# chto/linna

Measured on AMD Instinct MI355X. Metric: emulator log-likelihood evals/sec, higher is better.
Workload: dtype f32; 1 GPU; 33-D Gaussian, 4x512 MLP emulator (33->512x4->33), nwalkers=4096 batched log-likelihood per GPU (BASELINE configs[1]); nwalkers_per_gpu=4096, launch=direct launches, parallelism=walkers sharded, 1 rank(s), no data-path collective

## Files before the change

### include/linna_hip.h

```cpp
#ifndef LINNA_HIP_H
#define LINNA_HIP_H
#include <stddef.h>
#include <stdint.h>

#ifdef __cplusplus
extern "C" {
#endif

#define LINNA_ABI_VERSION 12

typedef struct linna_ctx linna_ctx_t;
typedef struct linna_net linna_net_t;
typedef struct linna_logprob linna_logprob_t;
typedef struct linna_graph linna_graph_t;

int linna_abi_version(void);
const char* linna_last_error(void);
#define LINNA_OK 0
#define LINNA_ERR_INVALID (-1)
#define LINNA_ERR_HIP (-2)
#define LINNA_ERR_UNSUPPORTED (-3)
#define LINNA_ERR_INTERNAL (-4)
int linna_debug_raise(int kind);
int linna_ctx_create(int device, linna_ctx_t** out);
// ... 119 lines not shown
    linna_colmap_t outmap;
    const float* S; int lds;
    const float* Ssym;
    const float* w;
    const float* gscale;
    float temperature;
    const float* Sfac;
} linna_logprob_desc_t;

int linna_logprob_create(linna_ctx_t* ctx, linna_net_t* net, const linna_logprob_desc_t* desc,
                         linna_logprob_t** out);
int linna_logprob_destroy(linna_logprob_t* lp);
int linna_weights_changed(linna_ctx_t* ctx);
#define LINNA_PRECISION_FP32 0
#define LINNA_PRECISION_BF16 1
int linna_logprob_set_precision(linna_logprob_t* lp, int precision);
int linna_logprob_precision(const linna_logprob_t* lp, int* out);
int linna_logprob_set_grad_precision(linna_logprob_t* lp, int precision);
int linna_logprob_grad_precision(const linna_logprob_t* lp, int* out);
int linna_engine_rows(int rows);
int linna_dense_tri(int mode);
int linna_serve_plain(int on);
int linna_serve_plain_sched(int hand);
int linna_program_plain(const linna_layer_t* layers, int nlayers, int in_size, int rows, int dense_nout);
int linna_logprob_serve_plain(linna_logprob_t* lp, int B, int* out);
int linna_logprob_grad_launches(linna_logprob_t* lp, int B, int* out);
int linna_slice_fusion(int mask);
int linna_program_describe(const linna_layer_t* layers, int nlayers, int in_size, int rows, int dense_nout, char* buf,
                           size_t n);
int linna_program_describe_grad_bf16(const linna_layer_t* layers, int nlayers, int in_size, int rows, char* buf, size_t n);
size_t linna_logprob_ws_bytes(const linna_logprob_t* lp, int B, int with_grad);
int linna_logprob_eval(linna_logprob_t* lp, const float* Z, int ldz, int B, void* ws, float* lnP,
                       float* THETA, int ldt, void* stream);
int linna_logprob_eval_if(linna_logprob_t* lp, const float* Z, int ldz, int B, void* ws, float* lnP,
                          float* THETA, int ldt, const int* gate, void* stream);
int linna_logprob_eval_slice_points(linna_logprob_t* lp, const float* coords, int ldc, int ndim, const int* S_idx,
                                    int ns, const float* DIR, int ldd, const float* w, int nrep, float* lnP,
                                    const int* gate, void* stream);
int linna_logprob_grad(linna_logprob_t* lp, const float* Z, int ldz, int B, void* ws, float* lnP,
                       float* G, int ldg, void* stream);
int linna_logprob_grad_leapfrog(linna_logprob_t* lp, float* Q, int ldq, int B, void* ws, float* lnP, float* G, int ldg,
                                float* P, int ldp, const float* mass, float eps_kick, float eps_drift, void* stream);

typedef struct {
    uint32_t struct_size;
    int nout;
// ... 165 lines not shown
```

### linna_amd/_lib.py

```python
import ctypes as C
import os

import torch

_HERE = os.path.dirname(os.path.abspath(__file__))
LIB_PATH = os.environ.get("LINNA_LIB_PATH") or os.path.join(_HERE, "liblinna_hip.so")
ABI_VERSION = 12

c_float_p = C.c_void_p
c_int_p = C.c_void_p


class _Sized(C.Structure):

    def __init__(self, *a, **k):
        C.Structure.__init__(self, *a, **k)
        self.struct_size = C.sizeof(type(self))


def sized_array(cls, n):
    arr = (cls * n)()
    for i in range(n):
        arr[i].struct_size = C.sizeof(cls)
    return arr
# ... 83 lines not shown
    "linna_net_create": (_I, [_V, C.POINTER(Layer), _I, _I, _PV]),
    "linna_net_destroy": (_I, [_V]),
    "linna_net_prepare": (_I, [_V, _I, _I]),
    "linna_net_fwd_ws_bytes": (_SZ, [_V, _I]),
    "linna_net_bwd_ws_bytes": (_SZ, [_V, _I]),
    "linna_net_forward": (_I, [_V, _V, _I, _I, _V, _V, _I, C.POINTER(ColMap), _V]),
    "linna_net_backward": (_I, [_V, _V, _I, _I, _V, _V, _V, _I, _V, _I, _I, _V]),
    "linna_net_stream_state": (_I, [_V, _V, _V, _V]),
    "linna_prior_map_fwd": (_I, [_V, _V, _I, _I, _I, _V, _V, _V, _V, _V, _V, _V, _I, _V, _I, _V]),
    "linna_prior_map_bwd": (_I, [_V, _V, _I, _I, _I, _V, _V, _V, _V, _V, _V, _I, _V, _I, _V]),
    "linna_gauss_loglike_diag": (_I, [_V, _V, _I, _I, _I, _V, _V, _I, _I, _F, _V, _V]),
    "linna_gauss_loglike_dense": (_I, [_V, _V, _I, _I, _I, _V, _I, _V, _I, _I, _F, _V, _V, _V]),
    "linna_logprob_create": (_I, [_V, _V, C.POINTER(LogprobDesc), _PV]),
    "linna_logprob_destroy": (_I, [_V]),
    "linna_weights_changed": (_I, [_V]),
    "linna_logprob_set_precision": (_I, [_V, _I]),
    "linna_logprob_precision": (_I, [_V, _V]),
    "linna_logprob_set_grad_precision": (_I, [_V, _I]),
    "linna_logprob_grad_precision": (_I, [_V, _V]),
    "linna_engine_rows": (_I, [_I]),
    "linna_dense_tri": (_I, [_I]),
    "linna_serve_plain": (_I, [_I]),
    "linna_serve_plain_sched": (_I, [_I]),
    "linna_program_plain": (_I, [_V, _I, _I, _I, _I]),
    "linna_logprob_serve_plain": (_I, [_V, _I, _V]),
    "linna_logprob_grad_launches": (_I, [_V, _I, _V]),
    "linna_slice_fusion": (_I, [_I]),
    "linna_net_train_launches": (_I, [_V, _I]),
    "linna_net_set_train_precision": (_I, [_V, _I]),
    "linna_net_train_precision": (_I, [_V, _V]),
    "linna_program_describe": (_I, [_V, _I, _I, _I, _I, _V, C.c_size_t]),
    "linna_program_describe_grad_bf16": (_I, [_V, _I, _I, _I, _V, C.c_size_t]),
    "linna_logprob_ws_bytes": (_SZ, [_V, _I, _I]),
    "linna_logprob_eval": (_I, [_V, _V, _I, _I, _V, _V, _V, _I, _V]),
    "linna_logprob_grad": (_I, [_V, _V, _I, _I, _V, _V, _V, _I, _V]),
    "linna_logprob_grad_leapfrog": (_I, [_V, _V, _I, _I, _V, _V, _V, _I, _V, _I, _V, _F, _F, _V]),
    "linna_loss_scratch_bytes": (_SZ, [_I, _I]),
    "linna_chi2_md": (_I, [_V, C.POINTER(LossDesc), _V, _I, _I, _V, _V, _V]),
    "linna_chi2_ratio_loss_fwd_bwd": (_I, [_V, C.POINTER(LossDesc), _V, _I, _V, _I, _V, _V, _I, _V, _V, _V, _V, _I, _F, _V]),
    "linna_net_prepare_loss": (_I, [_V, C.POINTER(LossDesc)]),
    "linna_loss_targets": (_I, [_V, C.POINTER(LossDesc), _V, _I, _I, _V, _I, _V]),
    "linna_net_forward_loss": (_I, [_V, C.POINTER(LossDesc), _V, _I, _V, _I, _V, _V, _V, _V, _I, _V, _V, _I, _V, _I, _V, _F, _V, _V, _V, _I,
                                    _V, _V, _F, _F, _V]),
    "linna_net_train_step": (_I, [_V, C.POINTER(LossDesc), _V, _I, _V, _I, _V, _V, _V, _V, _I, _V, _V, _I, _V, _I, _V, _F, _V, _V, _V, _I,
                                  _V, _V, _V, _F, _F, _V]),
    "linna_net_train_step_update": (_I, [_V, C.POINTER(LossDesc), _V, _I, _V, _I, _V, _V, _V, _V, _I, _V, _V, _I, _V, _I, _V, _F, _V, _V, _V, _I,
# ... 175 lines not shown
        return self

    def __exit__(self, *exc):
        import gc
        if self.on:
            gc.unfreeze()
        return False


def slice_fusion(mask=-1):
    prev = load().linna_slice_fusion(int(mask))
    if prev < 0:
        check(prev)
    return prev


def serve_plain_sched(hand=-1):
    prev = load().linna_serve_plain_sched(int(hand))
    if prev < 0:
        check(prev)
    return prev


def serve_plain(on=-1):
    prev = load().linna_serve_plain(int(on))
    if prev < 0:
        check(prev)
    return prev


def engine_rows(rows=0):
    prev = load().linna_engine_rows(int(rows))
    if prev < 0:
        check(prev)
    return prev
```

### linna_amd/csrc/api.hip

```cpp
#include "common.h"

#include <stdarg.h>
#include <stdio.h>
#include <string.h>
#include <cstring>
#include <string>
#include <vector>
#include <atomic>
#include <new>
#include <stdlib.h>

namespace linna {

static thread_local std::string g_err;

void set_error(const char* fmt, ...) {
    char buf[512];
    va_list ap;
    va_start(ap, fmt);
    vsnprintf(buf, sizeof buf, fmt, ap);
    va_end(ap);
    g_err = buf;
}

// ... 1033 lines not shown
int linna_program_describe_grad_bf16(const linna_layer_t* layers, int nlayers, int in_size, int rows, char* buf, size_t n) try {
    if (!layers || nlayers < 1 || !buf || !n) { set_error("program_describe_grad_bf16: bad arguments"); return LINNA_ERR_INVALID; }
    TRY(check_layers(layers, nlayers, "program_describe_grad_bf16"));
    return net_stream_describe(NS_GRAD_INPUT_BF16, layers, nlayers, in_size, nullptr, rows, buf, n);
} LINNA_CATCH_INT
int linna_program_describe(const linna_layer_t* layers, int nlayers, int in_size, int rows, int dense_nout, char* buf, size_t n) try {
    if (!layers || nlayers < 1 || !buf || !n) { set_error("program_describe: bad arguments"); return LINNA_ERR_INVALID; }
    TRY(check_layers(layers, nlayers, "program_describe"));
    static float dummy;
    if (dense_nout == -1) return net_stream_describe(ns_grad_kind(layers, nlayers), layers, nlayers, in_size, nullptr, rows, buf, n);
    const int dn_cols = dense_nout < -1 ? -dense_nout : dense_nout;
    NsDense dn{&dummy, (dn_cols + 3) & ~3, nullptr, nullptr, dense_nout < -1 ? 1 : 0, net_stream_dense_tri(-1)};
    if (dn_cols > 0) return net_stream_describe(NS_SERVE_DENSE, layers, nlayers, in_size, &dn, rows, buf, n);
    return net_stream_describe(NS_SERVE, layers, nlayers, in_size, nullptr, rows, buf, n);
} LINNA_CATCH_INT
int linna_serve_plain(int on) try {
    if (on < -1 || on > 1) { set_error("linna_serve_plain: %d (-1 query, 0 or 1)", on); return LINNA_ERR_INVALID; }
    return net_stream_serve_plain(on);
} LINNA_CATCH_INT
int linna_serve_plain_sched(int hand) try {
    if (hand < -1 || hand > 1) { set_error("linna_serve_plain_sched: %d (-1 query, 0 or 1)", hand); return LINNA_ERR_INVALID; }
    return net_stream_serve_plain_sched(hand);
} LINNA_CATCH_INT
int linna_program_plain(const linna_layer_t* layers, int nlayers, int in_size, int rows, int dense_nout) try {
    if (!layers || nlayers < 1) { set_error("program_plain: bad arguments"); return LINNA_ERR_INVALID; }
    TRY(check_layers(layers, nlayers, "program_plain"));
    if (dense_nout != 0) return 0;
    return net_stream_program_plain(NS_SERVE, layers, nlayers, in_size, nullptr, rows) ? 1 : 0;
} LINNA_CATCH_INT
int linna_logprob_serve_plain(linna_logprob_t* lp, int B, int* out) try {
    if (!lp || !out || B < 1) { set_error("logprob_serve_plain: bad arguments"); return LINNA_ERR_INVALID; }
    static float dummy[4];
    const LpRun r = lp_fused_run(lp, LpRun{dummy, 0, B, dummy}, dummy, LpLayout{});
    const NsDense dn = lp->dense();
    *out = !lp->bf16() && lp_serves_fused(lp, false) && !lp->dense_fused &&
           net_stream_takes_plain(lp->kind(), net_layers(lp->net, lp->kind()), lp_output(lp), r.lnP, r.D, r.TH, nullptr, nullptr, r.gate,
                                  net_stream_rows(B), lp->kind() == NS_SERVE_DENSE ? &dn : nullptr);
    return LINNA_OK;
} LINNA_CATCH_INT
int linna_dense_tri(int mode) try {
    if (mode < -1 || mode > 2) { set_error("linna_dense_tri: %d (-1 query, 0, 1 or 2)", mode); return LINNA_ERR_INVALID; }
    return net_stream_dense_tri(mode);
} LINNA_CATCH_INT
static std::atomic<int> g_slice_fusion{7};
static bool slice_derive_enabled() { return (g_slice_fusion.load() & 1) != 0; }
int linna_slice_fusion(int mode) try {
// ... 699 lines not shown
```

### linna_amd/csrc/common.h

```cpp
#pragma once
#include <hip/hip_runtime.h>
#include <stdint.h>
#include <exception>
#include "../../include/linna_hip.h"


typedef float f32x4 __attribute__((ext_vector_type(4)));
typedef float f32x16 __attribute__((ext_vector_type(16)));

namespace linna {

struct U4 { uint32_t x, y, z, w; };
__device__ __forceinline__ U4 philox4x32_10(U4 c, uint32_t k0, uint32_t k1) {
#pragma unroll
    for (int r = 0; r < 10; ++r) {
        const uint64_t p0 = (uint64_t)0xD2511F53u * c.x;
        const uint64_t p1 = (uint64_t)0xCD9E8D57u * c.z;
        U4 n;
        n.x = (uint32_t)(p1 >> 32) ^ c.y ^ k0;
        n.y = (uint32_t)p1;
        n.z = (uint32_t)(p0 >> 32) ^ c.w ^ k1;
        n.w = (uint32_t)p0;
        c = n;
        k0 += 0x9E3779B9u; k1 += 0xBB67AE85u;
// ... 266 lines not shown
    NS_SERVE_BF16,
    NS_STORE,
    NS_TRAIN_FWD,
    NS_DX,
    NS_DX_INPUT,
    NS_GRAD_INPUT,
    NS_TRAIN_STEP,
    NS_TRAIN_STEP_BF16,
    NS_GRAD_INPUT_BF16,
    NS_GRAD_INPUT_WIDE,
};
inline bool ns_kind_full_layers(NsKind k) { return k == NS_SERVE || k == NS_SERVE_DENSE || k == NS_SERVE_BF16; }
struct NsPlan { bool ok; size_t packed_floats; bool grad_ok; const char* why; };
NsPlan net_stream_plan(NsKind kind, const linna_layer_t* layers, int nl, int in_size, const NsDense* dn = nullptr);
int net_stream_rows(int B);
int net_stream_force_rows(int rows);
inline NsKind ns_grad_kind(const linna_layer_t* layers, int nl) { return nl >= 1 && layers[nl - 1].N > 64 ? NS_GRAD_INPUT_WIDE : NS_GRAD_INPUT; }
bool net_stream_grad_fits(const linna_layer_t* layers, int nl, int in_size, int rows);
int launch_net_stream_pack(NsKind kind, const linna_layer_t* layers, int nl, int in_size, float* packed, int rows, const NsDense* dn,
                           hipStream_t s);
int net_stream_describe(NsKind kind, const linna_layer_t* layers, int nl, int in_size, const NsDense* dn, int rows, char* buf, size_t n);
int net_stream_serve_plain(int on);
int net_stream_serve_plain_sched(int hand);
bool net_stream_program_plain(NsKind kind, const linna_layer_t* layers, int nl, int in_size, const NsDense* dn, int rows);
bool net_stream_launch_plain_ok(bool cscale, bool cshift, bool w, bool cexp, bool lnP, bool D, bool TH, bool gate);
struct NsNet { const linna_layer_t* layers; int nl, in_size; };
struct NsInput { int nin; const int* is_flat; const float* a1; const float* a2; const int* lg; const float* xmean; const float* xstd; };
struct NsOutput { const float* cscale; const float* cshift; const float* cpost; const float* cshift2; const float* w; float T; };
struct NsOpBufs { float* y; int ldy; float* t; int ldt; const float* x; int ldx; const float* gate; float* dprev; int ldp; float* dt; int lddt; };
struct NsPost { const float* rows; int n; float scale; float* out; int* step; float* hyper; float b1, b2; };
int launch_net_stream_dx(const NsNet& net, const float* packed, const float* dOUT, int lddo, int B, const NsOpBufs* ops, int with_input,
                         int rows, hipStream_t s, const NsPost* post = nullptr);
struct NsMove {
    float* coords; int ldc; float* logp; const int* S;
    const float* cc; int ldcc; const int* C; int nc;
    unsigned long long seed; const int* step; int step_off; int stream; float a; int* naccept;
    int slice;
    float* chain = nullptr; float* lps = nullptr;
    const float* sl_Z0 = nullptr; const float* sl_L = nullptr; const float* sl_R = nullptr; const float* sl_Zt = nullptr;
    int sl_m = 0, sl_nt = 0; unsigned long long sl_seed = 0; const int* sl_step = nullptr; int sl_stream = 0;
    const int* sl_flags = nullptr;
    const SliceBegin* sb = nullptr;
};
int launch_net_stream_store(const NsNet& net, const float* packed, const float* X, int ldx, int B, const NsOpBufs* ops,
                            const float* cscale, const float* cshift, int rows, hipStream_t s);
struct NsTrainLoss { const float* YN; int ldyn;
// ... 82 lines not shown
```

### linna_amd/csrc/net_program.hip

```cpp
#include "net_program.h"
#include <stdlib.h>
#include <algorithm>
#include <atomic>
#include <cstring>
#include <mutex>
#include <string>
#include <unordered_map>

namespace linna {

size_t NsProgram::lds_for(int rows, bool grad) const {
    size_t b = (size_t)(2 * rows * LD + ((bias_total + 3) & ~3)) * sizeof(float) + 128 + (x0_keep ? 4096 : 0);
#ifdef NS_STAMPS
    b += NS_NW * 32 * 8;
#endif
    return b + (grad ? (size_t)mask_slots * 64 * NS_NW * sizeof(unsigned) : 0);
}

static int ceil16(int k) { return (k + 15) & ~15; }
int ns_seg_steps(const NsSeg& s) {
    if (s.type == NS_WIDE && s.zext < 0) return 2 * s.steps - 60;
    return s.type == NS_WIDE && s.zext > 0 ? s.steps + (s.passes - 1) * s.zext : s.steps * s.passes;
}
static int ns_switch(std::atomic<int>& sw, const char* name, int dflt, bool (*valid)(int)) {
// ... 378 lines not shown
    cache.emplace(std::move(key), p);
    return p;
}

bool ns_program_plain(const NsProgram& p) {
    if (!p.ok || p.bf || p.dense || p.x0_keep || p.side_f4 || p.nseg_f < 1) return false;
    for (int i = 0; i < p.nseg_f; ++i) {
        const NsSeg& g = p.seg[i];
        if (g.type != NS_WIDE && g.type != NS_SPLIT) return false;
        if (g.x0_col || (g.type == NS_WIDE && (g.zext || g.kslice))) return false;
    }
    return true;
}
bool net_stream_program_plain(NsKind kind, const linna_layer_t* layers, int nl, int in_size, const NsDense* dn, int rows) {
    return kind == NS_SERVE && rows == 16 && ns_program_plain(*ns_program(kind, layers, nl, in_size, dn, rows));
}
bool net_stream_launch_plain_ok(bool cscale, bool cshift, bool w, bool cexp, bool lnP, bool D, bool TH, bool gate) {
    return cscale && cshift && w && !cexp && lnP && !D && !TH && !gate;
}
static std::atomic<int> g_serve_plain{1};
int net_stream_serve_plain(int on) { return on < 0 ? g_serve_plain.load() : g_serve_plain.exchange(on ? 1 : 0); }
static std::atomic<int> g_serve_plain_sched{1};
int net_stream_serve_plain_sched(int hand) { return hand < 0 ? g_serve_plain_sched.load() : g_serve_plain_sched.exchange(hand ? 1 : 0); }

int ns_seg_cols(const NsProgram& p, const linna_layer_t* layers, int i) {
    const linna_layer_t& l = layers[p.seg_op[i]];
    return p.seg_hidden[i] ? l.C : i < p.nseg_f ? l.N : l.K;
}
NsGates ns_gates(const NsProgram& p, const linna_layer_t* layers, int nl, int rows) {
    NsGates g;
    for (int i = 0; i < NS_MAXSEG; ++i) g.gbit[i] = g.mbit[i] = -1;
    for (int i = 0; i < p.nseg_f; ++i) {
        const int op = p.seg_op[i];
        if (op >= nl || (!p.seg_hidden[i] && op == nl - 1)) continue;
        g.gbit[i] = g.ncols;
        g.ncols += (ns_seg_cols(p, layers, i) + 63) & ~63;
    }
    for (int i = p.nseg_f; i < (int)p.seg.size(); ++i) {
        const int op = p.seg_op[i];
        const bool hidden = p.seg_hidden[i] != 0;
        if (!hidden && !(op > 0 && (layers[op - 1].op == LINNA_OP_RESBLOCK || layers[op - 1].relu))) continue;
        const int src = hidden ? op : op - 1;
        for (int j = 0; j < p.nseg_f; ++j)
            if (p.seg_op[j] == src && (p.seg_hidden[j] != 0) == hidden) g.mbit[i] = g.gbit[j];
        if (g.mbit[i] < 0) g.ok = false;
    }
// ... 188 lines not shown
```

### linna_amd/csrc/net_stream.hip

```cpp
#include "net_program.h"
#include <stdlib.h>
#include <type_traits>
#include <cstring>
#include <algorithm>

namespace linna {

typedef __bf16 bf16x8 __attribute__((ext_vector_type(8)));
typedef short s16x4 __attribute__((ext_vector_type(4)));

#ifndef NS_R
#define NS_R 6
#endif
#ifndef NS_PRE
#define NS_PRE 2
#endif
struct NsArgs {
    const float* Z; int ldz; int B; int nin;
    const int* is_flat; const float* a1; const float* a2; const int* lg;
    const float* xmean; const float* xstd;
    const float* packed;
    int G, nseg, LD, kpad0, nout, bias_total;
    int Gstride, nseg_f;
    const float* gscale; float* Gout; int ldg;
// ... 169 lines not shown
}
template <int R, int MOVE, bool GRAD, int STORE, int ROWS, bool BF, bool EPSV>
__global__ __launch_bounds__(64 * NS_NW, 1) void net_stream_wide_kernel(NsArgs a) {
    static_assert(!BF && GRAD && STORE == 2 && MOVE == 0, "the fp32 one-launch gradient of any network only");
    constexpr bool EPS = EPSV, PLAIN = false, WOUT = true;
#include "net_stream_body.inc"
}
template <int R>
__global__ __launch_bounds__(64 * NS_NW, 1) void net_stream_plain_kernel(NsArgs a) {
    constexpr int MOVE = 0, STORE = 0, ROWS = 16;
    constexpr bool GRAD = false, BF = false, EPS = false, PLAIN = true, WOUT = false;
#include "net_stream_body.inc"
}
#if NS_R == 6
#define NS_HAVE_PLACED 1
template <int R>
__global__ __launch_bounds__(64 * NS_NW, 1) void net_stream_placed_kernel(NsArgs a) {
    constexpr int MOVE = 0, STORE = 0, ROWS = 16;
    constexpr bool GRAD = false, BF = false, EPS = false, PLAIN = true, WOUT = false;
#define NS_BODY_HAND
#include "net_stream_body.inc"
#undef NS_BODY_HAND
}
#endif
template <int R, int MOVE, bool GRAD, int STORE, int ROWS, bool BF>
__global__ __launch_bounds__(64 * NS_NW, 1) void net_stream_train_bf16_kernel(NsArgs a) {
    static_assert(BF && GRAD && STORE == 3 && ROWS == 4 && MOVE == 0, "the bf16 training step only");
    constexpr bool EPS = false, PLAIN = false, WOUT = false;
#include "net_stream_body.inc"
}
template <int R, int MOVE, bool GRAD, int STORE, int ROWS, bool BF>
__global__ __launch_bounds__(64 * NS_NW, 1) void net_stream_slice_bf16_kernel(NsArgs a) {
    static_assert(BF && !GRAD && STORE == 0 && MOVE == 2, "the bf16 slice evaluation only");
    constexpr bool EPS = false, PLAIN = false, WOUT = false;
#define NS_BODY_SLICE_BF16
#include "net_stream_body.inc"
#undef NS_BODY_SLICE_BF16
}
template <int R, int MOVE, bool GRAD, int STORE, int ROWS, bool BF>
__global__ __launch_bounds__(64 * NS_NW, 1) void net_stream_grad_bf16_kernel(NsArgs a) {
    static_assert(BF && GRAD && STORE == 2 && MOVE == 0, "the bf16 one-launch gradient only");
    constexpr bool EPS = false, PLAIN = false, WOUT = false;
#define NS_BODY_GRAD_BF16
#include "net_stream_body.inc"
#undef NS_BODY_GRAD_BF16
}
// ... 46 lines not shown
    const size_t total = (size_t)NS_NW * p.Gstride * NS_NT * 64 + (size_t)p.bias_total;
    hipLaunchKernelGGL(ns_pack_kernel, dim3((unsigned)((total + 255) / 256)), dim3(256), 0, s, a);
    if (p.side_f4) hipLaunchKernelGGL(ns_pack_side_kernel, dim3((unsigned)((p.side_f4 + 255) / 256)), dim3(256), 0, s, a);
    return check_hip(hipGetLastError(), "net_stream pack launch");
}

template <void (*Kernel)(NsArgs)>
static int ns_launch(const NsArgs& a, int nblocks, size_t lds_bytes, hipStream_t s, const char* what) {
    static bool attr_set = false;
    if (!attr_set) {
        const int rc = check_hip(hipFuncSetAttribute(reinterpret_cast<const void*>(Kernel), hipFuncAttributeMaxDynamicSharedMemorySize, NS_LDS_BYTES),
                                 "hipFuncSetAttribute");
        if (rc != LINNA_OK) return rc;
        attr_set = true;
    }
    hipLaunchKernelGGL(Kernel, dim3(nblocks), dim3(64 * NS_NW), lds_bytes, s, a);
    return check_hip(hipGetLastError(), what);
}
template <int MOVE, bool GRAD, int STORE, int ROWS, bool BF = false, bool EPS = false>
static int ns_launch_rows(const NsArgs& a, int B, size_t lds_bytes, hipStream_t s, int extra = 0) {
    if constexpr (EPS) return ns_launch<net_stream_eps_kernel<NS_R, MOVE, GRAD, STORE, ROWS, BF>>(a, (B + ROWS - 1) / ROWS + extra, lds_bytes, s, "net_stream launch");
    else return ns_launch<net_stream_kernel<NS_R, MOVE, GRAD, STORE, ROWS, BF>>(a, (B + ROWS - 1) / ROWS + extra, lds_bytes, s, "net_stream launch");
}
template <int MOVE, bool GRAD, int STORE = 0, bool BF = false, bool EPS = false>
static int ns_launch_kernel(const NsArgs& a0, int B, const NsProgram& p, int rows, hipStream_t s, int extra = 0, size_t lds_extra = 0,
                            bool plain = false, bool wide = false) {
    const size_t lds = p.lds_for(rows, GRAD) + lds_extra;
#ifdef NS_STAMPS
    NsArgs a = a0;
    a.stamps = getenv("LINNA_FUSED_STAMPS") ? reinterpret_cast<unsigned long long*>(strtoull(getenv("LINNA_FUSED_STAMPS"), nullptr, 16)) : nullptr;
    if (!a.stamps) { set_error("net_stream: NS_STAMPS build needs LINNA_FUSED_STAMPS"); return LINNA_ERR_INVALID; }
#else
    const NsArgs& a = a0;
#endif
    if constexpr (MOVE == 0 && !GRAD && STORE == 0 && !BF && !EPS) {
#ifdef NS_HAVE_PLACED
        if (plain && rows == 16 && net_stream_serve_plain_sched(-1))
            return ns_launch<net_stream_placed_kernel<NS_R>>(a, (B + 15) / 16, lds, s, "net_stream plain launch (hand-placed step)");
#endif
        if (plain && rows == 16) return ns_launch<net_stream_plain_kernel<NS_R>>(a, (B + 15) / 16, lds, s, "net_stream plain launch");
    }
    if constexpr (MOVE == 0 && GRAD && STORE == 2 && !BF) {
        const char* const what = "net_stream wide-output gradient launch";
        if (wide && rows == 4) return ns_launch<net_stream_wide_kernel<NS_R, 0, true, 2, 4, false, EPS>>(a, (B + 3) / 4, lds, s, what);
        if (wide && rows == 8) return ns_launch<net_stream_wide_kernel<NS_R, 0, true, 2, 8, false, EPS>>(a, (B + 7) / 8, lds, s, what);
        if (wide && rows == 16) return ns_launch<net_stream_wide_kernel<NS_R, 0, true, 2, 16, false, EPS>>(a, (B + 15) / 16, lds, s, what);
    }
    if (rows == 4) return ns_launch_rows<MOVE, GRAD, STORE, 4, BF, EPS>(a, B, lds, s, extra);
    if constexpr (BF) {
        if (rows == 8) return ns_launch_rows<MOVE, GRAD, STORE, 8, BF, EPS>(a, B, lds, s, extra);
        if (rows == 16) return ns_launch_rows<MOVE, GRAD, STORE, 16, BF, EPS>(a, B, lds, s, extra);
    } else if constexpr (STORE == 3 && GRAD) {
    } else {
        if (rows == 8) return ns_launch_rows<MOVE, GRAD, STORE, 8, false, EPS>(a, B, lds, s, extra);
        if (rows == 16) return ns_launch_rows<MOVE, GRAD, STORE, 16, false, EPS>(a, B, lds, s, extra);
    }
    set_error("net_stream: %d rows per workgroup", rows);
    return LINNA_ERR_INVALID;
}
// ... 334 lines not shown
```

### linna_amd/csrc/net_stream_body.inc

```
    constexpr int NT = NS_NT, NW = NS_NW;
    constexpr int RG = 32;
    constexpr bool SM = ROWS < 16;
    constexpr int RS = SM ? ROWS / 4 : 1;
    constexpr int NQ = SM ? RS : NT;
    constexpr int NACC = SM ? 4 * RS : NT;
#ifdef NS_BODY_SLICE_BF16
    static_assert(BF && !GRAD && STORE == 0 && MOVE == 2, "bf16: the slice evaluation");
#elif defined(NS_BODY_GRAD_BF16)
    static_assert(BF && GRAD && STORE == 2 && MOVE == 0, "bf16: lnP and its gradient in one launch");
#else
    static_assert(!BF || (!GRAD && STORE == 0 && MOVE != 2) || (GRAD && STORE == 3 && MOVE == 0 && ROWS == 4),
                  "bf16: serving, the fused stretch move and the merged training step (4-row engine)");
#endif
    constexpr bool BFT = BF && GRAD && STORE == 3;
    constexpr int AK = BF ? 2 : 1;
    constexpr bool K4 = !SM && !BF && (STORE == 0 || (GRAD && STORE == 2));
    constexpr bool TRB = GRAD && STORE == 3;
    constexpr bool DXE = STORE == 2 || TRB;
    constexpr bool G2 = GRAD && STORE == 2;
    constexpr bool LB = G2;
    constexpr bool LATE_REFILL = true;
#ifdef NS_BODY_HAND
    constexpr bool HAND = true;
    static_assert(PLAIN && !BF && ROWS == 16 && R == 6 && NS_NT == 4 && LATE_REFILL, "the hand-placed step: plain fp32 serving, 16 rows, six slots");
#else
    constexpr bool HAND = false;
#endif
#define NS_HAND_RING \
    "+{v[128:131]}"(Bq[0][0]), "+{v[132:135]}"(Bq[0][1]), "+{v[136:139]}"(Bq[0][2]), "+{v[140:143]}"(Bq[0][3]), \
    "+{v[144:147]}"(Bq[1][0]), "+{v[148:151]}"(Bq[1][1]), "+{v[152:155]}"(Bq[1][2]), "+{v[156:159]}"(Bq[1][3]), \
    "+{v[160:163]}"(Bq[2][0]), "+{v[164:167]}"(Bq[2][1]), "+{v[168:171]}"(Bq[2][2]), "+{v[172:175]}"(Bq[2][3]), \
    "+{v[176:179]}"(Bq[3][0]), "+{v[180:183]}"(Bq[3][1]), "+{v[184:187]}"(Bq[3][2]), "+{v[188:191]}"(Bq[3][3]), \
    "+{v[192:195]}"(Bq[4][0]), "+{v[196:199]}"(Bq[4][1]), "+{v[200:203]}"(Bq[4][2]), "+{v[204:207]}"(Bq[4][3]), \
    "+{v[208:211]}"(Bq[5][0]), "+{v[212:215]}"(Bq[5][1]), "+{v[216:219]}"(Bq[5][2]), "+{v[220:223]}"(Bq[5][3])
#define NS_HAND_A "+{v[224:227]}"(Aq[0][0]), "+{v[228:231]}"(Aq[1][0])
#define NS_HAND_ACC "+{v[232:235]}"(acc[0]), "+{v[236:239]}"(acc[1]), "+{v[240:243]}"(acc[2]), "+{v[244:247]}"(acc[3])
    constexpr bool RNAN = STORE == 1;
    auto relu_f = [](float v) { if constexpr (RNAN) return isnan(v) ? v : fmaxf(v, 0.f); else return fmaxf(v, 0.f); };
    static_assert(ROWS == 16 || ROWS == 8 || ROWS == 4, "rows per workgroup");
    static_assert(R % 2 == 0, "the A double buffer alternates with the ring slot parity");
    extern __shared__ __attribute__((aligned(16))) float smem[];
    const int LD = a.LD, ABUF = ROWS * LD;
    constexpr bool KA = STORE == 3 || STORE == 1 || GRAD;
    const NsArgs* const ka = KA ? reinterpret_cast<const NsArgs*>((const void*)__builtin_amdgcn_kernarg_segment_ptr()) : &a;
    float* const act = smem;
    float* const lbias = smem + 2 * ABUF;
    unsigned* const lbits = reinterpret_cast<unsigned*>(smem + a.bits_off);
    const int nbw = a.nbw;
    const int tid = threadIdx.x, lane = tid & 63;
// ... 359 lines not shown
    auto gstore = [&](float* p, float v) { asm volatile("global_store_dword %0, %1, off" :: "v"(p), "v"(v) : "memory"); };
    uint32_t ap;
    auto a_read = [&](f32x4* dst) {
        if constexpr (HAND) {
            if (dst == Aq[0]) asm volatile("ds_read_b128 %0, %1" : "={v[224:227]}"(Aq[0][0]) : "v"(ap) : "memory");
            else asm volatile("ds_read_b128 %0, %1" : "={v[228:231]}"(Aq[1][0]) : "v"(ap) : "memory");
        } else
        asm volatile("ds_read_b128 %0, %1" : "=v"(dst[0]) : "v"(ap) : "memory");
        if constexpr (BF) asm volatile("ds_read_b128 %0, %1 offset:16" : "=v"(dst[1]) : "v"(ap) : "memory");
        if constexpr (BFT) ap += si == a.nseg_f - 1 ? 64 : 64 * AK;
        else ap += 64 * AK;
    };
    auto load_seg = [&]() {
        const NsSeg S = ka->seg[__builtin_amdgcn_readfirstlane(si)];
        s_type = S.type; kleft = s_steps = S.steps; s_passes = S.passes; s_bias = S.bias_off;
        s_dst = S.dst_col; s_relu = S.relu; s_kslice = S.kslice; s_zext = S.zext; s_ncgl = S.ncg_log2; s_x0col = S.x0_col; s_x0n = S.x0_n;
        if constexpr (GRAD) { s_mstore = S.mask_store; s_mapply = S.mask_apply; }
        if constexpr (STORE) { const int j = __builtin_amdgcn_readfirstlane(si); s_gout = ka->gout[j]; s_gld = ka->gld[j]; s_gn = ka->gn[j]; }
        if constexpr (DXE) { const int j = __builtin_amdgcn_readfirstlane(si); s_gmask = ka->gmask[j]; s_gmld = ka->gmld[j]; }
        if constexpr (LB) { const int j = __builtin_amdgcn_readfirstlane(si); s_gbit = ka->gbit[j]; s_mbit = ka->mbit[j]; }
    };
    NsSeg nxp;
    auto plain_request = [&]() { nxp = ka->seg[__builtin_amdgcn_readfirstlane(min(si + 1, nseg - 1))]; };
    auto plain_take = [&](const NsSeg& X) {
        s_type = X.type & 255; s_ncgl = X.type >> 8; kleft = s_steps = X.steps; s_passes = X.passes; s_bias = X.bias_off;
        s_dst = X.dst_col; s_relu = X.relu; s_kslice = X.kslice; s_zext = X.zext;
    };
    auto begin_run = [&]() {
        const int arow = SM ? sm_arow : li, ak = AK * (SM ? 4 * sm_achunk : 4 * kq);
#pragma unroll
        for (int t = 0; t < NACC; ++t) acc[t] = f32x4{0.f, 0.f, 0.f, 0.f};
        if (s_type == NS_WIDE) {
            const int blk = !PLAIN && s_zext < 0 ? (pass ? 15 - wave : wave) : 8 * pass + wave;
            if constexpr (SM) {
                const float b = lbias[s_bias + 64 * blk + lane];
#pragma unroll
                for (int r = 0; r < RS; ++r) acc[4 * r] = f32x4{b, b, b, b};
            } else {
#pragma unroll
                for (int t = 0; t < NT; ++t) {
                    const float b = lbias[s_bias + 16 * (4 * blk + t) + li];
                    acc[t] = f32x4{b, b, b, b};
                }
            }
            if (!PLAIN && s_zext < 0) kleft = s_steps - 4 * blk;
            ap = act_lds + 4u * (uint32_t)(P * ABUF + arow * LD + ak + (PLAIN ? 0 : s_zext < 0 ? 64 * blk : (pass ? s_kslice : 0)));
        } else {
            ap = act_lds + 4u * (uint32_t)(P * ABUF + arow * LD + ak + (wave >> s_ncgl) * s_kslice);
        }
        if constexpr (BFT) {
            if (si == a.nseg_f - 1) ap -= 4u * (uint32_t)(ak / 2);
        }
        if constexpr (HAND) asm volatile("s_nop 3" : NS_HAND_ACC);
    };
    auto lds_barrier = [&]() {
        asm volatile("s_waitcnt lgkmcnt(0)" ::: "memory");
        __builtin_amdgcn_s_barrier();
        asm volatile("" ::: "memory");
    };
    if constexpr (PLAIN) {
        asm volatile("" :: "s"(seg_warm));
        plain_take(ka->seg[0]); begin_run(); a_read(Aq[0]); plain_request();
    }
    else {
    load_seg();
    begin_run();
    a_read(Aq[0]);
    }

    auto step = [&](auto Uc, auto Refill) {
        constexpr int U = decltype(Uc)::value;
        constexpr bool refill = decltype(Refill)::value;
        constexpr int RU = LATE_REFILL ? (U + R - 1) % R : U;
        if constexpr (HAND) {
            constexpr int BU = 128 + 16 * U, BR = 128 + 16 * RU, AC = 224 + 4 * (U & 1), AN = 224 + 4 * ((U + 1) & 1);
            constexpr int TW = refill ? 0 : 4 * U;
#define NS_HM(t, s) "v_mfma_f32_16x16x4_f32 v[232+4*" #t ":235+4*" #t "], v[%[ac]+" #s "], v[%[bu]+4*" #t "+" #s "], v[232+4*" #t ":235+4*" #t "]\n\t"
#define NS_HL(t, off) "global_load_dwordx4 v[%[ru]+4*" #t ":%[ru]+4*" #t "+3], %[vo], %[sb] offset:" #off "\n\t"
#define NS_HAND_TEXT(HEAD, L0, L1, L2, L3) HEAD \
            "s_waitcnt lgkmcnt(0)\n\t" \
            "s_waitcnt vmcnt(%[w0])\n\t" \
            NS_HM(0, 0) "ds_read_b128 v[%[an]:%[an]+3], %[ap]\n\t" \
            "s_waitcnt vmcnt(%[w1])\n\t" \
            NS_HM(1, 0) \
            NS_HM(0, 1) L0 \
            NS_HM(1, 1) \
            NS_HM(0, 2) L1 \
            NS_HM(1, 2) \
            NS_HM(0, 3) L2 \
            NS_HM(1, 3) \
            "s_waitcnt vmcnt(%[w2])\n\t" \
            NS_HM(2, 0) L3 \
            "s_waitcnt vmcnt(%[w3])\n\t" \
            NS_HM(3, 0) \
            NS_HM(2, 1) "v_add_u32 %[ap], 64, %[ap]\n\t" \
            NS_HM(3, 1) NS_HM(2, 2) NS_HM(3, 2) NS_HM(2, 3) NS_HM(3, 3)
            if constexpr (refill) {
                const char* const sb = wbase + woff;
#ifdef NS_HAND_PHASE4
#define NS_HAND_HEAD ".p2align 3\n\ts_nop 0\n\t"
#else
#define NS_HAND_HEAD ".p2align 3\n\t"
#endif
                if constexpr (U == 0)
                    asm volatile(NS_HAND_TEXT(NS_HAND_HEAD, NS_HL(0, 0), NS_HL(1, 1024), NS_HL(2, 2048), NS_HL(3, 3072))
                                 : NS_HAND_RING, NS_HAND_A, NS_HAND_ACC, [ap] "+v"(ap)
                                 : [vo] "v"(voff), [sb] "s"(sb), [bu] "n"(BU), [ru] "n"(BR), [ac] "n"(AC), [an] "n"(AN),
                                   [w0] "n"(19), [w1] "n"(18), [w2] "n"(20), [w3] "n"(20) : "memory");
                else
                    asm volatile(NS_HAND_TEXT("", NS_HL(0, 0), NS_HL(1, 1024), NS_HL(2, 2048), NS_HL(3, 3072))
                                 : NS_HAND_RING, NS_HAND_A, NS_HAND_ACC, [ap] "+v"(ap)
                                 : [vo] "v"(voff), [sb] "s"(sb), [bu] "n"(BU), [ru] "n"(BR), [ac] "n"(AC), [an] "n"(AN),
                                   [w0] "n"(19), [w1] "n"(18), [w2] "n"(20), [w3] "n"(20) : "memory");
                wadvance();
            } else {
                asm volatile(NS_HAND_TEXT("", "", "", "", "")
                             : NS_HAND_RING, NS_HAND_A, NS_HAND_ACC, [ap] "+v"(ap)
                             : [bu] "n"(BU), [ac] "n"(AC), [an] "n"(AN),
                               [w0] "n"(19 - TW), [w1] "n"(18 - TW), [w2] "n"(17 - TW), [w3] "n"(16 - TW) : "memory");
            }
#undef NS_HAND_TEXT
#undef NS_HAND_HEAD
#undef NS_HL
#undef NS_HM
        } else {
        if constexpr (BF) asm volatile("s_waitcnt lgkmcnt(0)" : "+v"(Aq[U & 1][0]), "+v"(Aq[U & 1][AK - 1]) :: "memory");
        else asm volatile("s_waitcnt lgkmcnt(0)" : "+v"(Aq[U & 1][0]) :: "memory");
        a_read(Aq[(U + 1) & 1]);
        const f32x4 av = Aq[U & 1][0];
        if constexpr (BF) {
            bf16x8 ab;
#pragma unroll
            for (int e = 0; e < 4; ++e) { ab[e] = (__bf16)Aq[U & 1][0][e]; ab[4 + e] = (__bf16)Aq[U & 1][AK - 1][e]; }
            if constexpr (SM) {
                auto bf_small = [&]() {
                    const s16x4 alo = __builtin_bit_cast(s16x4, __builtin_shufflevector(ab, ab, 0, 1, 2, 3));
                    const s16x4 ahi = __builtin_bit_cast(s16x4, __builtin_shufflevector(ab, ab, 4, 5, 6, 7));
#define NS_B4(r, c, h, A4) acc[4 * (r) + (c)] = __builtin_amdgcn_mfma_f32_4x4x4bf16_1k(A4, \
                __builtin_bit_cast(s16x4, __builtin_shufflevector(__builtin_bit_cast(bf16x8, Bq[U][c]), __builtin_bit_cast(bf16x8, Bq[U][c]), \
                                                                  4 * (h), 4 * (h) + 1, 4 * (h) + 2, 4 * (h) + 3)), acc[4 * (r) + (c)], 4, 4 * (c) + (r), 0);
#define NS_B4R(r, h, A4) NS_B4(r, 0, h, A4) NS_B4(r, 1, h, A4) NS_B4(r, 2, h, A4) NS_B4(r, 3, h, A4)
                    NS_B4R(0, 0, alo)
                    if constexpr (RS > 1) { NS_B4R(1, 0, alo) }
                    NS_B4R(0, 1, ahi)
// ... 568 lines not shown
#ifdef NS_STAMPS_FINE
                    if (fine) { asm volatile("s_waitcnt lgkmcnt(0)" ::: "memory"); NS_STAMP(); }
#endif
                    lds_barrier();
                    NS_STAMP();
                    ++si;
                    const int n2i = __builtin_amdgcn_readfirstlane(min(si, nseg - 1));
                    const NsSeg N2 = ka->seg[n2i];
                    take_seg(N2);
                    if constexpr (LB) { s_gbit = ka->gbit[n2i]; s_mbit = ka->mbit[n2i]; s_gn = ka->gn[n2i]; }
                }
            }
            if (si < nseg) {
                begin_run();
                a_read(Aq[(U + 1) & 1]);
                if constexpr (PLAIN) { if (seg_done) plain_request(); }
            }
#ifdef NS_STAMPS_FINE
            if (fine) { asm volatile("s_waitcnt lgkmcnt(0)" ::: "memory"); NS_STAMP(); }
#endif
        }
    };
    using T_ = std::true_type; using F_ = std::false_type;
#define NS_STEP(U, RF) if constexpr (U < R) step(std::integral_constant<int, U>{}, RF{});
    const int ngroups = a.G / R, rem = a.G - ngroups * R;
#pragma unroll 1
    for (int it = 0; it < ngroups; ++it) {
        NS_STEP(0, T_) NS_STEP(1, T_) NS_STEP(2, T_) NS_STEP(3, T_) NS_STEP(4, T_) NS_STEP(5, T_) NS_STEP(6, T_) NS_STEP(7, T_)
    }
#define NS_TAIL(U) if constexpr (U < R - 1) { if (rem > U) step(std::integral_constant<int, U>{}, F_{}); }
    NS_TAIL(0) NS_TAIL(1) NS_TAIL(2) NS_TAIL(3) NS_TAIL(4) NS_TAIL(5) NS_TAIL(6)
#undef NS_STEP
#undef NS_TAIL
    if constexpr (BF) asm volatile("s_waitcnt lgkmcnt(0)" : "+v"(Aq[0][0]), "+v"(Aq[0][AK - 1]), "+v"(Aq[1][0]), "+v"(Aq[1][AK - 1]) :: "memory");
    else asm volatile("s_waitcnt lgkmcnt(0)" : "+v"(Aq[0][0]), "+v"(Aq[1][0]) :: "memory");
    NS_STAMP();

    if constexpr (((STORE == 1 || STORE == 2) && !GRAD) || TRB) { NS_STAMPS_FLUSH(); return; }
    if constexpr (STORE == 3) {
        const float* const F = act + P * ABUF + pr * LD;
        const bool rok = prow && row0 + pr < a.B;
        const float* const Dv = a.u_same ? F : act + (P ^ 1) * ABUF + pr * LD;
        const float* const Uv = a.u_same ? F + a.u_col : F;
        float chi = 0.f;
        for (int c = pc0; c < nout; c += RG) chi += Dv[c] * Uv[c];
#pragma unroll
        for (int o = RG / 2; o >= 1; o >>= 1) chi += __shfl_xor(chi, o, 64);
        if (rok && pc0 == 0) a.t_loss_rows[row0 + pr] = chi / lden[pr];
        {
            constexpr int TPR = 64 * NW / ROWS;
            const int fr = tid / TPR, fc = tid % TPR;
            if (row0 + fr < a.B) {
                const float* const Fr = act + P * ABUF + fr * LD;
                const float* const Dr = a.u_same ? Fr : act + (P ^ 1) * ABUF + fr * LD;
                const float* const Ur = a.u_same ? Fr + a.u_col : Fr;
// ... 116 lines not shown
```

Before: 76.35 million evals/s.

## Skip padded MFMA tiles in first and last segments of hand-placed plain kernel

Adds a trimmed variant of the hand-placed fp32 serving kernel that masks off MFMA instructions covering padding. Columns beyond nout in the final split segment are skipped, as are K-chunks beyond the real input width in the first segment's last step. The main loop is split into head, middle and tail groups so only the boundary iterations carry the scalar branch-and-mask code. It is enabled by default through a new toggle. This adds scalar branches inside the hand-scheduled asm and larger code size for the boundary steps.

```diff
diff --git a/include/linna_hip.h b/include/linna_hip.h
--- a/include/linna_hip.h
+++ b/include/linna_hip.h
@@ -165,6 +165,7 @@
 int linna_dense_tri(int mode);
 int linna_serve_plain(int on);
 int linna_serve_plain_sched(int hand);
+int linna_serve_plain_trim(int on);
 int linna_program_plain(const linna_layer_t* layers, int nlayers, int in_size, int rows, int dense_nout);
 int linna_logprob_serve_plain(linna_logprob_t* lp, int B, int* out);
 int linna_logprob_grad_launches(linna_logprob_t* lp, int B, int* out);
diff --git a/linna_amd/_lib.py b/linna_amd/_lib.py
--- a/linna_amd/_lib.py
+++ b/linna_amd/_lib.py
@@ -129,6 +129,7 @@
     "linna_dense_tri": (_I, [_I]),
     "linna_serve_plain": (_I, [_I]),
     "linna_serve_plain_sched": (_I, [_I]),
+    "linna_serve_plain_trim": (_I, [_I]),
     "linna_program_plain": (_I, [_V, _I, _I, _I, _I]),
     "linna_logprob_serve_plain": (_I, [_V, _I, _V]),
     "linna_logprob_grad_launches": (_I, [_V, _I, _V]),
@@ -350,6 +351,13 @@
     return prev
 
 
+def serve_plain_trim(on=-1):
+    prev = load().linna_serve_plain_trim(int(on))
+    if prev < 0:
+        check(prev)
+    return prev
+
+
 def serve_plain(on=-1):
     prev = load().linna_serve_plain(int(on))
     if prev < 0:
diff --git a/linna_amd/csrc/api.hip b/linna_amd/csrc/api.hip
--- a/linna_amd/csrc/api.hip
+++ b/linna_amd/csrc/api.hip
@@ -1079,6 +1079,10 @@
     if (hand < -1 || hand > 1) { set_error("linna_serve_plain_sched: %d (-1 query, 0 or 1)", hand); return LINNA_ERR_INVALID; }
     return net_stream_serve_plain_sched(hand);
 } LINNA_CATCH_INT
+int linna_serve_plain_trim(int on) try {
+    if (on < -1 || on > 1) { set_error("linna_serve_plain_trim: %d (-1 query, 0 or 1)", on); return LINNA_ERR_INVALID; }
+    return net_stream_serve_plain_trim(on);
+} LINNA_CATCH_INT
 int linna_program_plain(const linna_layer_t* layers, int nlayers, int in_size, int rows, int dense_nout) try {
     if (!layers || nlayers < 1) { set_error("program_plain: bad arguments"); return LINNA_ERR_INVALID; }
     TRY(check_layers(layers, nlayers, "program_plain"));
diff --git a/linna_amd/csrc/common.h b/linna_amd/csrc/common.h
--- a/linna_amd/csrc/common.h
+++ b/linna_amd/csrc/common.h
@@ -312,6 +312,7 @@
 int net_stream_describe(NsKind kind, const linna_layer_t* layers, int nl, int in_size, const NsDense* dn, int rows, char* buf, size_t n);
 int net_stream_serve_plain(int on);
 int net_stream_serve_plain_sched(int hand);
+int net_stream_serve_plain_trim(int on);
 bool net_stream_program_plain(NsKind kind, const linna_layer_t* layers, int nl, int in_size, const NsDense* dn, int rows);
 bool net_stream_launch_plain_ok(bool cscale, bool cshift, bool w, bool cexp, bool lnP, bool D, bool TH, bool gate);
 struct NsNet { const linna_layer_t* layers; int nl, in_size; };
diff --git a/linna_amd/csrc/net_program.hip b/linna_amd/csrc/net_program.hip
--- a/linna_amd/csrc/net_program.hip
+++ b/linna_amd/csrc/net_program.hip
@@ -424,6 +424,8 @@
 int net_stream_serve_plain(int on) { return on < 0 ? g_serve_plain.load() : g_serve_plain.exchange(on ? 1 : 0); }
 static std::atomic<int> g_serve_plain_sched{1};
 int net_stream_serve_plain_sched(int hand) { return hand < 0 ? g_serve_plain_sched.load() : g_serve_plain_sched.exchange(hand ? 1 : 0); }
+static std::atomic<int> g_serve_plain_trim{1};
+int net_stream_serve_plain_trim(int on) { return on < 0 ? g_serve_plain_trim.load() : g_serve_plain_trim.exchange(on ? 1 : 0); }
 
 int ns_seg_cols(const NsProgram& p, const linna_layer_t* layers, int i) {
     const linna_layer_t& l = layers[p.seg_op[i]];
diff --git a/linna_amd/csrc/net_stream.hip b/linna_amd/csrc/net_stream.hip
--- a/linna_amd/csrc/net_stream.hip
+++ b/linna_amd/csrc/net_stream.hip
@@ -215,6 +215,16 @@
 #include "net_stream_body.inc"
 #undef NS_BODY_HAND
 }
+template <int R>
+__global__ __launch_bounds__(64 * NS_NW, 1) void net_stream_trimmed_kernel(NsArgs a) {
+    constexpr int MOVE = 0, STORE = 0, ROWS = 16;
+    constexpr bool GRAD = false, BF = false, EPS = false, PLAIN = true, WOUT = false;
+#define NS_BODY_HAND
+#define NS_BODY_TRIM
+#include "net_stream_body.inc"
+#undef NS_BODY_TRIM
+#undef NS_BODY_HAND
+}
 #endif
 template <int R, int MOVE, bool GRAD, int STORE, int ROWS, bool BF>
 __global__ __launch_bounds__(64 * NS_NW, 1) void net_stream_train_bf16_kernel(NsArgs a) {
@@ -307,6 +317,17 @@
     if constexpr (EPS) return ns_launch<net_stream_eps_kernel<NS_R, MOVE, GRAD, STORE, ROWS, BF>>(a, (B + ROWS - 1) / ROWS + extra, lds_bytes, s, "net_stream launch");
     else return ns_launch<net_stream_kernel<NS_R, MOVE, GRAD, STORE, ROWS, BF>>(a, (B + ROWS - 1) / ROWS + extra, lds_bytes, s, "net_stream launch");
 }
+static bool ns_plain_trims(const NsArgs& a) {
+    const NsSeg& l = a.seg[a.nseg - 1];
+    if ((l.type & 255) == NS_SPLIT && (l.type >> 8) == 0 && a.nout <= 48) return true;
+    const NsSeg& f = a.seg[0];
+    const int nkp = (f.type & 255) == NS_WIDE ? 1 : NS_NW >> (f.type >> 8);
+    for (int w = 0; w < nkp; ++w) {
+        const int real = a.nin - (((f.type & 255) == NS_WIDE ? 0 : w * f.kslice) + 16 * (f.steps - 1));
+        if (real > 0 && real < 4) return true;
+    }
+    return false;
+}
 template <int MOVE, bool GRAD, int STORE = 0, bool BF = false, bool EPS = false>
 static int ns_launch_kernel(const NsArgs& a0, int B, const NsProgram& p, int rows, hipStream_t s, int extra = 0, size_t lds_extra = 0,
                             bool plain = false, bool wide = false) {
@@ -320,6 +341,8 @@
 #endif
     if constexpr (MOVE == 0 && !GRAD && STORE == 0 && !BF && !EPS) {
 #ifdef NS_HAVE_PLACED
+        if (plain && rows == 16 && net_stream_serve_plain_sched(-1) && net_stream_serve_plain_trim(-1) && ns_plain_trims(a))
+            return ns_launch<net_stream_trimmed_kernel<NS_R>>(a, (B + 15) / 16, lds, s, "net_stream plain launch (hand-placed step, short forms)");
         if (plain && rows == 16 && net_stream_serve_plain_sched(-1))
             return ns_launch<net_stream_placed_kernel<NS_R>>(a, (B + 15) / 16, lds, s, "net_stream plain launch (hand-placed step)");
 #endif
diff --git a/linna_amd/csrc/net_stream_body.inc b/linna_amd/csrc/net_stream_body.inc
--- a/linna_amd/csrc/net_stream_body.inc
+++ b/linna_amd/csrc/net_stream_body.inc
@@ -25,6 +25,12 @@
     static_assert(PLAIN && !BF && ROWS == 16 && R == 6 && NS_NT == 4 && LATE_REFILL, "the hand-placed step: plain fp32 serving, 16 rows, six slots");
 #else
     constexpr bool HAND = false;
+#endif
+#ifdef NS_BODY_TRIM
+    constexpr bool TRIM = true;
+    static_assert(HAND, "the short step texts belong to the hand-placed step");
+#else
+    constexpr bool TRIM = false;
 #endif
 #define NS_HAND_RING \
     "+{v[128:131]}"(Bq[0][0]), "+{v[132:135]}"(Bq[0][1]), "+{v[136:139]}"(Bq[0][2]), "+{v[140:143]}"(Bq[0][3]), \
@@ -430,9 +436,25 @@
     };
     NsSeg nxp;
     auto plain_request = [&]() { nxp = ka->seg[__builtin_amdgcn_readfirstlane(min(si + 1, nseg - 1))]; };
+    int s_tlim = 0; unsigned s_ntm = 0xFFFFu, s_kcm = 0xFFFFu;
+    auto trim_setup = [&]() {
+        s_tlim = 0; s_ntm = 0xFFFFu; s_kcm = 0xFFFFu;
+        if (si == nseg - 1 && s_type == NS_SPLIT && s_ncgl == 0 && nout <= 48) {
+            s_ntm = (1u << (4 * ((nout + 15) >> 4))) - 1u;
+            s_tlim = 0x7FFFFFFF;
+        }
+        if (si == 0) {
+            const int real = nin - ((s_type == NS_WIDE ? 0 : (wave >> s_ncgl) * s_kslice) + 16 * (s_steps - 1));
+            if (real > 0 && real < 4) {
+                s_kcm = 0x1111u * ((1u << real) - 1u);
+                s_tlim = max(s_tlim, 1);
+            }
+        }
+    };
     auto plain_take = [&](const NsSeg& X) {
         s_type = X.type & 255; s_ncgl = X.type >> 8; kleft = s_steps = X.steps; s_passes = X.passes; s_bias = X.bias_off;
         s_dst = X.dst_col; s_relu = X.relu; s_kslice = X.kslice; s_zext = X.zext;
+        if constexpr (TRIM) trim_setup();
     };
     auto begin_run = [&]() {
         const int arow = SM ? sm_arow : li, ak = AK * (SM ? 4 * sm_achunk : 4 * kq);
@@ -476,33 +498,48 @@
     a_read(Aq[0]);
     }
 
-    auto step = [&](auto Uc, auto Refill) {
+    auto step = [&](auto Uc, auto Refill, auto Mixed) {
         constexpr int U = decltype(Uc)::value;
         constexpr bool refill = decltype(Refill)::value;
+        constexpr bool mixed = TRIM && decltype(Mixed)::value;
         constexpr int RU = LATE_REFILL ? (U + R - 1) % R : U;
         if constexpr (HAND) {
             constexpr int BU = 128 + 16 * U, BR = 128 + 16 * RU, AC = 224 + 4 * (U & 1), AN = 224 + 4 * ((U + 1) & 1);
             constexpr int TW = refill ? 0 : 4 * U;
 #define NS_HM(t, s) "v_mfma_f32_16x16x4_f32 v[232+4*" #t ":235+4*" #t "], v[%[ac]+" #s "], v[%[bu]+4*" #t "+" #s "], v[232+4*" #t ":235+4*" #t "]\n\t"
 #define NS_HL(t, off) "global_load_dwordx4 v[%[ru]+4*" #t ":%[ru]+4*" #t "+3], %[vo], %[sb] offset:" #off "\n\t"
-#define NS_HAND_TEXT(HEAD, L0, L1, L2, L3) HEAD \
+#define NS_HAND_TEXT(M, HEAD, L0, L1, L2, L3) HEAD \
             "s_waitcnt lgkmcnt(0)\n\t" \
             "s_waitcnt vmcnt(%[w0])\n\t" \
             NS_HM(0, 0) "ds_read_b128 v[%[an]:%[an]+3], %[ap]\n\t" \
             "s_waitcnt vmcnt(%[w1])\n\t" \
-            NS_HM(1, 0) \
-            NS_HM(0, 1) L0 \
-            NS_HM(1, 1) \
-            NS_HM(0, 2) L1 \
-            NS_HM(1, 2) \
-            NS_HM(0, 3) L2 \
-            NS_HM(1, 3) \
+            M(1, 0) \
+            M(0, 1) L0 \
+            M(1, 1) \
+            M(0, 2) L1 \
+            M(1, 2) \
+            M(0, 3) L2 \
+            M(1, 3) \
             "s_waitcnt vmcnt(%[w2])\n\t" \
-            NS_HM(2, 0) L3 \
+            M(2, 0) L3 \
             "s_waitcnt vmcnt(%[w3])\n\t" \
-            NS_HM(3, 0) \
-            NS_HM(2, 1) "v_add_u32 %[ap], 64, %[ap]\n\t" \
-            NS_HM(3, 1) NS_HM(2, 2) NS_HM(3, 2) NS_HM(2, 3) NS_HM(3, 3)
+            M(3, 0) \
+            M(2, 1) "v_add_u32 %[ap], 64, %[ap]\n\t" \
+            M(3, 1) M(2, 2) M(3, 2) M(2, 3) M(3, 3)
+#define NS_HG(t, s) "s_bitcmp0_b32 %[mk], 4*" #t "+" #s "\n\ts_cbranch_scc1 .Lns_skip_%=_" #t #s "\n\t" NS_HM(t, s) ".Lns_skip_%=_" #t #s ":\n\t"
+#define NS_TRIM_TEXT(HEAD, L0, L1, L2, L3) HEAD \
+            "s_cmp_le_i32 %[kl], %[tl]\n\t" \
+            "s_cbranch_scc1 .Lns_short_%=\n\t" \
+            NS_HAND_TEXT(NS_HM, "", L0, L1, L2, L3) \
+            "s_branch .Lns_end_%=\n" \
+            ".Lns_short_%=:\n\t" \
+            "s_cmp_eq_u32 %[kl], 1\n\t" \
+            "s_cselect_b32 %[mk], %[kcm], 0xffff\n\t" \
+            "s_and_b32 %[mk], %[mk], %[ntm]\n\t" \
+            NS_HAND_TEXT(NS_HG, "", L0, L1, L2, L3) \
+            ".Lns_end_%=:\n\t"
+#define NS_TRIM_OPS [kl] "s"(kleft), [tl] "s"(s_tlim), [kcm] "s"(s_kcm), [ntm] "s"(s_ntm)
+            unsigned mk;
             if constexpr (refill) {
                 const char* const sb = wbase + woff;
 #ifdef NS_HAND_PHASE4
@@ -510,24 +547,43 @@
 #else
 #define NS_HAND_HEAD ".p2align 3\n\t"
 #endif
-                if constexpr (U == 0)
-                    asm volatile(NS_HAND_TEXT(NS_HAND_HEAD, NS_HL(0, 0), NS_HL(1, 1024), NS_HL(2, 2048), NS_HL(3, 3072))
+                if constexpr (mixed && U == 0)
+                    asm volatile(NS_TRIM_TEXT(NS_HAND_HEAD, NS_HL(0, 0), NS_HL(1, 1024), NS_HL(2, 2048), NS_HL(3, 3072))
+                                 : NS_HAND_RING, NS_HAND_A, NS_HAND_ACC, [ap] "+v"(ap), [mk] "=&s"(mk)
+                                 : [vo] "v"(voff), [sb] "s"(sb), [bu] "n"(BU), [ru] "n"(BR), [ac] "n"(AC), [an] "n"(AN),
+                                   [w0] "n"(19), [w1] "n"(18), [w2] "n"(20), [w3] "n"(20), NS_TRIM_OPS : "memory", "scc");
+                else if constexpr (mixed)
+                    asm volatile(NS_TRIM_TEXT("", NS_HL(0, 0), NS_HL(1, 1024), NS_HL(2, 2048), NS_HL(3, 3072))
+                                 : NS_HAND_RING, NS_HAND_A, NS_HAND_ACC, [ap] "+v"(ap), [mk] "=&s"(mk)
+                                 : [vo] "v"(voff), [sb] "s"(sb), [bu] "n"(BU), [ru] "n"(BR), [ac] "n"(AC), [an] "n"(AN),
+                                   [w0] "n"(19), [w1] "n"(18), [w2] "n"(20), [w3] "n"(20), NS_TRIM_OPS : "memory", "scc");
+                else if constexpr (U == 0)
+                    asm volatile(NS_HAND_TEXT(NS_HM, NS_HAND_HEAD, NS_HL(0, 0), NS_HL(1, 1024), NS_HL(2, 2048), NS_HL(3, 3072))
                                  : NS_HAND_RING, NS_HAND_A, NS_HAND_ACC, [ap] "+v"(ap)
                                  : [vo] "v"(voff), [sb] "s"(sb), [bu] "n"(BU), [ru] "n"(BR), [ac] "n"(AC), [an] "n"(AN),
                                    [w0] "n"(19), [w1] "n"(18), [w2] "n"(20), [w3] "n"(20) : "memory");
                 else
-                    asm volatile(NS_HAND_TEXT("", NS_HL(0, 0), NS_HL(1, 1024), NS_HL(2, 2048), NS_HL(3, 3072))
+                    asm volatile(NS_HAND_TEXT(NS_HM, "", NS_HL(0, 0), NS_HL(1, 1024), NS_HL(2, 2048), NS_HL(3, 3072))
                                  : NS_HAND_RING, NS_HAND_A, NS_HAND_ACC, [ap] "+v"(ap)
                                  : [vo] "v"(voff), [sb] "s"(sb), [bu] "n"(BU), [ru] "n"(BR), [ac] "n"(AC), [an] "n"(AN),
                                    [w0] "n"(19), [w1] "n"(18), [w2] "n"(20), [w3] "n"(20) : "memory");
                 wadvance();
+            } else if constexpr (mixed) {
+                asm volatile(NS_TRIM_TEXT("", "", "", "", "")
+                             : NS_HAND_RING, NS_HAND_A, NS_HAND_ACC, [ap] "+v"(ap), [mk] "=&s"(mk)
+                             : [bu] "n"(BU), [ac] "n"(AC), [an] "n"(AN),
+                               [w0] "n"(19 - TW), [w1] "n"(18 - TW), [w2] "n"(17 - TW), [w3] "n"(16 - TW), NS_TRIM_OPS : "memory", "scc");
             } else {
-                asm volatile(NS_HAND_TEXT("", "", "", "", "")
+                asm volatile(NS_HAND_TEXT(NS_HM, "", "", "", "", "")
                              : NS_HAND_RING, NS_HAND_A, NS_HAND_ACC, [ap] "+v"(ap)
                              : [bu] "n"(BU), [ac] "n"(AC), [an] "n"(AN),
                                [w0] "n"(19 - TW), [w1] "n"(18 - TW), [w2] "n"(17 - TW), [w3] "n"(16 - TW) : "memory");
             }
+            (void)mk;
+#undef NS_TRIM_OPS
+#undef NS_TRIM_TEXT
 #undef NS_HAND_TEXT
+#undef NS_HG
 #undef NS_HAND_HEAD
 #undef NS_HL
 #undef NS_HM
@@ -1142,15 +1198,30 @@
         }
     };
     using T_ = std::true_type; using F_ = std::false_type;
-#define NS_STEP(U, RF) if constexpr (U < R) step(std::integral_constant<int, U>{}, RF{});
+#define NS_STEP(U, RF, MX) if constexpr (U < R) step(std::integral_constant<int, U>{}, RF{}, MX{});
+#define NS_GROUP(MX) NS_STEP(0, T_, MX) NS_STEP(1, T_, MX) NS_STEP(2, T_, MX) NS_STEP(3, T_, MX) NS_STEP(4, T_, MX) NS_STEP(5, T_, MX) \
+    NS_STEP(6, T_, MX) NS_STEP(7, T_, MX)
     const int ngroups = a.G / R, rem = a.G - ngroups * R;
+    if constexpr (TRIM) {
+        const NsSeg s0 = ka->seg[0], sl = ka->seg[__builtin_amdgcn_readfirstlane(nseg - 1)];
+        const int nhead = min((s0.steps * s0.passes + R - 1) / R, ngroups);
+        const int ntail = max((a.G - sl.steps * sl.passes) / R, nhead);
+#pragma unroll 1
+        for (int it = 0; it < nhead; ++it) { NS_GROUP(T_) }
+#pragma unroll 1
+        for (int it = nhead; it < ntail; ++it) { NS_GROUP(F_) }
+#pragma unroll 1
+        for (int it = ntail; it < ngroups; ++it) { NS_GROUP(T_) }
+    } else {
 #pragma unroll 1
     for (int it = 0; it < ngroups; ++it) {
-        NS_STEP(0, T_) NS_STEP(1, T_) NS_STEP(2, T_) NS_STEP(3, T_) NS_STEP(4, T_) NS_STEP(5, T_) NS_STEP(6, T_) NS_STEP(7, T_)
-    }
-#define NS_TAIL(U) if constexpr (U < R - 1) { if (rem > U) step(std::integral_constant<int, U>{}, F_{}); }
+        NS_GROUP(F_)
+    }
+    }
+#define NS_TAIL(U) if constexpr (U < R - 1) { if (rem > U) step(std::integral_constant<int, U>{}, F_{}, T_{}); }
     NS_TAIL(0) NS_TAIL(1) NS_TAIL(2) NS_TAIL(3) NS_TAIL(4) NS_TAIL(5) NS_TAIL(6)
 #undef NS_STEP
+#undef NS_GROUP
 #undef NS_TAIL
     if constexpr (BF) asm volatile("s_waitcnt lgkmcnt(0)" : "+v"(Aq[0][0]), "+v"(Aq[0][AK - 1]), "+v"(Aq[1][0]), "+v"(Aq[1][AK - 1]) :: "memory");
     else asm volatile("s_waitcnt lgkmcnt(0)" : "+v"(Aq[0][0]), "+v"(Aq[1][0]) :: "memory");
```

Result: no change. 75.60 million evals/s (-1.0%).
